# stevenabreu7/SparseRNNs

Measured on AMD Instinct MI355X. Metric: frames/sec at w8a16 S5 dim_scale=0.5 (NDNS shape), bit-exact vs CPU fxprun, higher is better.
Workload: dtype int32

## Files before the change

### include/s5fxp.h

```cpp
#ifndef S5FXP_H
#define S5FXP_H

#include <stddef.h>
#include <stdint.h>

#ifdef __cplusplus
extern "C" {
#endif

#define S5FXP_VERSION 115

enum {
    S5FXP_OK = 0,
    S5FXP_EBADARG = -1,
    S5FXP_ENEGSHIFT = -2,
    S5FXP_EUNSUPPORTED = -3,
    S5FXP_EHIP = -4,
    S5FXP_EWORKSPACE = -5
};

enum { S5FXP_FLOOR = 0, S5FXP_CEIL = 1, S5FXP_ROUND = 2 };

int s5fxp_version(void);
const char *s5fxp_strerror(int code);
// ... 114 lines not shown
typedef struct {
    s5fxp_norm_desc norm;
    s5fxp_ssm_desc ssm;
    s5fxp_dense_desc out2;
    int32_t l_bits, l_exp, r_bits, r_exp, res_bits, res_exp;
    int32_t sig_x_exp, sig_y_exp;
    int32_t lut[8];
} s5fxp_layer_desc;

typedef struct {
    int32_t n_layers;
    s5fxp_dense_desc encoder;
    const s5fxp_layer_desc *layers;
    s5fxp_dense_desc decoder;
} s5fxp_model_desc;

typedef struct s5fxp_model s5fxp_model;

typedef struct {
    int32_t *pre_s5;
    int32_t *u;
    int32_t *Bu_re, *Bu_im;
    int32_t *xs_re, *xs_im;
    int32_t *ys;
    int32_t *out2;
    int32_t *out2_sigmoid;
    int32_t *post_GLU;
    int32_t *residadd;
} s5fxp_layer_trace;

size_t s5fxp_model_blob_bytes(const s5fxp_model_desc *desc);

enum { S5FXP_MODEL_DEFAULT = 0, S5FXP_MODEL_FORCE_DENSE = 1, S5FXP_MODEL_FORCE_CSR = 2, S5FXP_MODEL_FORCE_GENERIC = 4,
       S5FXP_MODEL_NO_RESID_FOLD = 8, S5FXP_MODEL_NO_RESID_LAZY = 16, S5FXP_MODEL_NO_GATE_EXT = 32 };
int s5fxp_model_create(const s5fxp_model_desc *desc, void *dev_blob, size_t blob_bytes, int flags, void *stream,
                       s5fxp_model **out);
void s5fxp_model_destroy(s5fxp_model *m);

size_t s5fxp_workspace_bytes(const s5fxp_model *m, int B, int L);

#define S5FXP_STATUS_WORDS 128
enum { S5FXP_PATH_GENERIC = 1, S5FXP_PATH_FUSED = 2, S5FXP_PATH_STEP = 3, S5FXP_PATH_CLIP = 4 };
enum {
    S5FXP_ST_NEGSHIFT = 1,
    S5FXP_ST_NEGEXP = 2,
    S5FXP_ST_WIDE_STATE = 4,
    S5FXP_ST_WIDE_INPUT = 8,
    S5FXP_ST_REDO = 16
};

enum { S5FXP_FWD_DEFER_REDO = 1, S5FXP_FWD_EXACT = 2, S5FXP_FWD_NO_PAIR = 4 };

typedef int (*s5fxp_allreduce_max_fn)(void *ctx, float *dev_vals, int n, void *stream);

typedef struct {
    s5fxp_allreduce_max_fn allreduce;
    void *allreduce_ctx;
    void **scan_events;
    int32_t flags;
    const int32_t *state_in;
    int32_t *state_out;
    int32_t groups;
    void **gate_events;
} s5fxp_forward_opts;

int s5fxp_model_forward(const s5fxp_model *m, const int32_t *x, int x_bits, int x_exp, int B, int L, int32_t *y,
                        void *workspace, size_t workspace_bytes, int32_t *status, const s5fxp_layer_trace *traces,
// ... 102 lines not shown
```

### sparsernns_amd/_lib.py

```python
from __future__ import annotations

import ctypes as C
import os

import torch

_HERE = os.path.dirname(os.path.abspath(__file__))
LIB_PATH = os.environ.get("S5FXP_LIB") or os.path.join(_HERE, "libs5fxp.so")

I32P = C.POINTER(C.c_int32)
VOIDP = C.c_void_p

S5FXP_OK, S5FXP_EBADARG, S5FXP_ENEGSHIFT, S5FXP_EUNSUPPORTED, S5FXP_EHIP, S5FXP_EWORKSPACE = 0, -1, -2, -3, -4, -5
ST_NEGSHIFT, ST_NEGEXP, ST_WIDE_STATE, ST_WIDE_INPUT, ST_REDO = 1, 2, 4, 8, 16
FWD_DEFER_REDO, FWD_EXACT, FWD_NO_PAIR = 1, 2, 4
STATUS_WORDS = 128
PATH_GENERIC, PATH_FUSED, PATH_STEP, PATH_CLIP = 1, 2, 3, 4
STEP_MAX_ROWS = 32
STREAM_MAX_HOPS = 32
PUSH_FRESH, PUSH_ZEROS, PUSH_FINAL = 1, 2, 4
MODEL_DEFAULT, MODEL_FORCE_DENSE, MODEL_FORCE_CSR, MODEL_FORCE_GENERIC, MODEL_NO_RESID_FOLD, MODEL_NO_RESID_LAZY = 0, 1, 2, 4, 8, 16
MODEL_NO_GATE_EXT = 32


class DenseDesc(C.Structure):
    _fields_ = [("K", C.c_int32), ("M", C.c_int32), ("weight", I32P), ("bias", I32P)] + [
        (n, C.c_int32) for n in ("w_bits", "w_exp", "b_bits", "b_exp", "inp_bits", "inp_exp", "out_bits", "out_exp")]


class SSMDesc(C.Structure):
    _fields_ = [("H", C.c_int32), ("P", C.c_int32)] + [
        (n, I32P) for n in ("A_re", "A_im", "B_re", "B_im", "C_re", "C_im", "D")] + [
        (n, C.c_int32) for n in (
            "A_re_bits", "A_re_exp", "A_im_bits", "A_im_exp", "B_re_bits", "B_re_exp", "B_im_bits", "B_im_exp",
            "C_re_bits", "C_re_exp", "C_im_bits", "C_im_exp", "D_bits", "D_exp",
            "u_bits", "u_exp", "Bu_re_bits", "Bu_re_exp", "Bu_im_bits", "Bu_im_exp",
            "x_re_bits", "x_re_exp", "x_im_bits", "x_im_exp", "y_bits", "y_exp")]


class NormDesc(C.Structure):
    _fields_ = [(n, I32P) for n in ("minus_mean", "invsq_var", "scale", "bias")] + [
        (n, C.c_int32) for n in ("mean_bits", "mean_exp", "invsq_var_bits", "invsq_var_exp", "scale_bits",
                                 "scale_exp", "bias_bits", "bias_exp")]


class LayerDesc(C.Structure):
    _fields_ = [("norm", NormDesc), ("ssm", SSMDesc), ("out2", DenseDesc)] + [
        (n, C.c_int32) for n in ("l_bits", "l_exp", "r_bits", "r_exp", "res_bits", "res_exp", "sig_x_exp",
                                 "sig_y_exp")] + [("lut", C.c_int32 * 8)]


class ModelDesc(C.Structure):
    _fields_ = [("n_layers", C.c_int32), ("encoder", DenseDesc), ("layers", C.POINTER(LayerDesc)),
                ("decoder", DenseDesc)]

# ... 158 lines not shown
```

### sparsernns_amd/csrc/mfma_bn.hpp

```cpp
#pragma once
#include "mfma_proj.hpp"

namespace s5 {

struct StatusInit {
    int32_t path;
    int32_t rk[15];
    int32_t slots[15];
    int32_t stream[15];
};
__global__ __launch_bounds__(256) void k_clear2(int32_t *a, int na, int32_t *b, int nb, StatusInit si, int n_layers, GroupOff go)
{
    gshift(a, (int64_t)blockIdx.y * go.status);
    gshift(b, (int64_t)blockIdx.y * go.ws);
    for (int i = blockIdx.x * 256 + threadIdx.x; i < na + nb; i += gridDim.x * 256) {
        if (i < na) {
            int32_t v = 0;
            if (i == 2) v = si.path;
            else if (i >= 8 && (i & 7) == 5 && (i - 8) / 8 < n_layers) v = si.rk[(i - 8) / 8];
            else if (i >= 8 && (i & 7) == 6 && (i - 8) / 8 < n_layers) v = si.slots[(i - 8) / 8];
            else if (i >= 8 && (i & 7) == 7 && (i - 8) / 8 < n_layers) v = si.stream[(i - 8) / 8];
            a[i] = v;
        } else b[i - na] = 0;
    }
// ... 681 lines not shown
{
    v4i u;
#pragma unroll
    for (int k = 0; k < 4; ++k) {
        if constexpr (ARM == ROW_GENERIC) {
            int32_t o[2];
#pragma unroll
            for (int e = 0; e < 2; ++e) {
                const int32_t xe = e ? x[k] >> 16 : (int32_t)(int16_t)(x[k] & 0xffff);
                const int32_t me = e ? (int32_t)p.m[k] >> 16 : (int32_t)(int16_t)(p.m[k] & 0xffffu);
                const int32_t ie = e ? (int32_t)p.iv[k] >> 16 : (int32_t)(int16_t)(p.iv[k] & 0xffffu);
                const int32_t v = sat(asr(wshl(wadd(sat(wshl(xe, p.shx1), p.xb), me), p.l1), p.r1), p.b1);
                const int32_t t = sat(asr(__mul24(v, ie), p.rs2), p.b2);
                o[e] = sat(asr(wshl(t, p.cl), p.cr), p.cbits);
            }
            u[k] = (int32_t)(((uint32_t)o[0] & 0xffffu) | ((uint32_t)o[1] << 16));
        } else {
            const uint32_t xs = pk_mul_sat_u((uint32_t)x[k], p.mulx);
            int32_t t0, t1;
            if constexpr (ARM == ROW_PACKED) {
                const uint32_t v = pk_add_sat(xs, p.m[k]);
                t0 = mul24_hh<0>(v, p.iv[k]); t1 = mul24_hh<1>(v, p.iv[k]);
            } else {
                const int32_t v0 = asr(add_hh<0>(xs, p.m[k]), p.r1), v1 = asr(add_hh<1>(xs, p.m[k]), p.r1);
                t0 = mul24_h<0>(v0, p.iv[k]); t1 = mul24_h<1>(v1, p.iv[k]);
            }
            const uint32_t t = pk_cvt(asr(t0, p.rs2), asr(t1, p.rs2));
            u[k] = (int32_t)pk_ashr_u(pk_mul_sat_u(t, p.mulc), p.crp);
        }
    }
    return u;
}

struct BprojM2Args {
    BnArgs bn;
    const int16_t *x;
    MfmaW w;
    int32_t *bq;
    int16_t *u;
    int32_t *tr_bu_re, *tr_bu_im, *tr_pre_s5, *tr_u;
    int64_t N;
    int32_t L, TB, H, P;
    int32_t rs_re, rs_im, bre_bits, bim_bits, sh_re, sh_im;
    int32_t t_lo, t_len;
    int32_t k_re;
    int32_t no_u;
    int32_t live_slots;
    const float *ext;
    int32_t ext_reps;
    int32_t *status, *status_exps;
    const LayerDyn *lazy;
};

}
```

### sparsernns_amd/csrc/proj_p.hpp

```cpp
#pragma once
#ifdef S5_PHASE_PROF
__device__ long long g_phase_prof[2048 * 8];
#define PHASE_DECL unsigned prof_last, prof_a0 = 0, prof_a1 = 0, prof_a2 = 0, prof_a3 = 0, prof_a4 = 0, prof_a5 = 0, prof_a6 = 0, prof_a7 = 0; \
    { unsigned long long t_; asm volatile("s_memtime %0\n\ts_waitcnt lgkmcnt(0)" : "=s"(t_)); prof_last = __builtin_amdgcn_readfirstlane((unsigned)t_); }
#define PHASE_MARK(i, reg) do { unsigned long long t_; asm volatile("v_cmp_eq_u32 vcc, %1, %1\n\ts_nop 0\n\ts_memtime %0\n\ts_waitcnt lgkmcnt(0)" : "=s"(t_) : "v"(reg) : "memory", "vcc"); \
    const unsigned tl_ = __builtin_amdgcn_readfirstlane((unsigned)t_); prof_a##i = __builtin_amdgcn_readfirstlane(prof_a##i + (tl_ - prof_last)); prof_last = tl_; } while (0)
#define PHASE_DUMP do { if (threadIdx.x == 0 && blockIdx.x < 2048) { long long *o_ = g_phase_prof + blockIdx.x * 8; o_[0] = prof_a0; o_[1] = prof_a1; o_[2] = prof_a2; o_[3] = prof_a3; \
    o_[4] = prof_a4; o_[5] = prof_a5; o_[6] = prof_a6; o_[7] = prof_a7; } } while (0)
#else
#define PHASE_DECL
#define PHASE_MARK(i, reg)
#define PHASE_DUMP
#endif
#include "mfma_bn.hpp"

namespace s5 {

__host__ __device__ constexpr int shape_channels(int NT) { return (NT == 2 || NT == 5) ? 32 * NT - 16 : 32 * NT; }

template <int HC, int HP, int KP>
__device__ __forceinline__ void zero_plane_tail(int8_t *base, int rows)
{
    if constexpr (HC != HP) {
        static_assert(HP - HC == 16, "half a tile");
        for (int i = threadIdx.x; i < rows; i += blockDim.x) *reinterpret_cast<v4i *>(base + i * KP + HC) = v4i{0, 0, 0, 0};
    }
}

__device__ __forceinline__ void planes8_from_i32(const int32_t (&v)[8], v2i &hi, v2i &lo)
{
#pragma unroll
    for (int j = 0; j < 2; ++j) {
        const unsigned p01 = perm((unsigned)v[4 * j + 1], (unsigned)v[4 * j], 0x05010400u);
        const unsigned p23 = perm((unsigned)v[4 * j + 3], (unsigned)v[4 * j + 2], 0x05010400u);
        lo[j] = (int)(perm(p23, p01, 0x05040100u) ^ 0x80808080u);
        hi[j] = (int)perm(p23, p01, 0x07060302u);
    }
}

struct StepRange {
    int32_t t_lo, t_len;
};
template <int FT = 64>
__device__ __forceinline__ void tile_of(int64_t tile, const StepRange &sr, int64_t &b, int &t, int &nvalid)
{
    const int tps = (sr.t_len + FT - 1) / FT;
    b = tile / tps;
    const int tt = (int)(tile - b * tps) * FT;
    t = sr.t_lo + tt;
    nvalid = sr.t_len - tt < FT ? sr.t_len - tt : FT;
}

template <int FT = 64>
struct TileWalk {
    int tps, db, dti;
    int b, ti;
    __device__ __forceinline__ TileWalk(int64_t tile0, const StepRange &sr, unsigned step)
    {
        tps = (sr.t_len + FT - 1) / FT;
        db = (int)(step / (unsigned)tps); dti = (int)(step % (unsigned)tps);
        b = (int)((unsigned)tile0 / (unsigned)tps); ti = (int)((unsigned)tile0 % (unsigned)tps);
    }
    __device__ __forceinline__ void advance()
    {
        b += db; ti += dti;
        if (ti >= tps) { ti -= tps; ++b; }
    }
    __device__ __forceinline__ TileWalk next() const { TileWalk n = *this; n.advance(); return n; }
    __device__ __forceinline__ int t(const StepRange &sr) const { return sr.t_lo + ti * FT; }
// ... 24 lines not shown
    const int wct = wave % NC, wsub = wave / NC;
    const StepRange sr{a.t_lo, a.t_len};
    const int64_t tiles = (a.N / a.L) * ((sr.t_len + FT - 1) / FT);
    int64_t tile = blockIdx.x;

    v4i raw[NV];
    auto fetch = [&](const TileWalk<FT> &tw) {
        const int64_t b = tw.b;
        const int t = tw.t(sr), nv = tw.nvalid(sr);
        const char *xb = reinterpret_cast<const char *>(a.x + (b * a.L + t) * H);
#pragma unroll
        for (int i = 0; i < NV; ++i) {
            const int v = threadIdx.x + NTHR * i;
            int f = v / VPF;
            f = f < nv ? f : nv - 1;
            raw[i] = *reinterpret_cast<const v4i *>(xb + 2u * (unsigned)(f * H + 8 * (v % VPF)));
        }
    };
    TileWalk<FT> walk(tile, sr, gridDim.x);
    if (tile < tiles) fetch(walk);
    v4i wreg[NCT][KS];
    int32_t csv[NCT];
#pragma unroll
    for (int c = 0; c < NCT; ++c) {
        const int col = 32 * (wct + NC * c) + r;
        csv[c] = a.w.cs128[col];
#pragma unroll
        for (int ks = 0; ks < KS; ++ks)
            wreg[c][ks] = *reinterpret_cast<const v4i *>(a.w.wt + (size_t)col * a.w.Kp + 32 * ks + 16 * h);
    }
    const LayerDyn d = a.ext ? bn_finalize_mm_body(a.bn, a.ext, H, const_cast<LayerDyn *>(a.bn.dyn), a.status, a.status_exps, a.bn.xe.get(), a.ext_reps,
                                                   blockIdx.x == 0)
                             : *a.bn.dyn;
    const Bn16 bn = bn16_setup(a.bn, d, tab, H);
    constexpr bool LAZY = KS == 3 && !TRACE;
    ResolveU16 rz{};
    int lazy_arm = 0;
    if constexpr (LAZY) {
        if (a.lazy) {
            gshift_nn(a.lazy, (int64_t)blockIdx.y * go.ws);
            rz = resolve_u16_setup(a.lazy->res.post);
            lazy_arm = 1 + rz.arm;
        }
    }
    __syncthreads();

    prologue_loads_done();
    for (int it = 0; tile < tiles; tile += gridDim.x, ++it, walk.advance()) {
        const int64_t b0 = walk.b;
        const int t0 = walk.t(sr), nvalid = walk.nvalid(sr);
        const int64_t n0 = b0 * a.L + t0;
        char *ub = reinterpret_cast<char *>(a.u + n0 * H);
        int8_t *xh = Xh + (it & 1) * PLANE, *xl = Xl + (it & 1) * PLANE;
#pragma unroll
        for (int i = 0; i < NV; ++i) {
            const int v = threadIdx.x + NTHR * i, f = v / VPF, og = v % VPF;
            const int64_t n = n0 + f;
            int32_t xin[8], t[8], u[8];
            if constexpr (LAZY) {
                if (lazy_arm == 1 + RES_RIGHT) {
#pragma unroll
                    for (int e = 0; e < 4; ++e) raw[i][e] = (int)resolve_u16_pair<RES_RIGHT>(rz, (uint32_t)raw[i][e]);
                } else if (lazy_arm) {
#pragma unroll
                    for (int e = 0; e < 4; ++e) raw[i][e] = (int)resolve_u16_pair<RES_GENERIC>(rz, (uint32_t)raw[i][e]);
                }
            }
            unpack8_i16(raw[i], xin);
            bn16_x4(bn, reinterpret_cast<const int32_t(&)[4]>(xin[0]), 8 * og, reinterpret_cast<int32_t(&)[4]>(t[0]),
                    reinterpret_cast<int32_t(&)[4]>(u[0]));
            bn16_x4(bn, reinterpret_cast<const int32_t(&)[4]>(xin[4]), 8 * og + 4, reinterpret_cast<int32_t(&)[4]>(t[4]),
                    reinterpret_cast<int32_t(&)[4]>(u[4]));
            if (f < nvalid && (TRACE || !a.no_u)) {
                const v2i p0 = pack4_i16(u[0], u[1], u[2], u[3]), p1 = pack4_i16(u[4], u[5], u[6], u[7]);
                *reinterpret_cast<v4i *>(ub + 2u * (unsigned)(f * H + 8 * og)) = v4i{p0[0], p0[1], p1[0], p1[1]};
                if (TRACE) {
#pragma unroll
                    for (int e = 0; e < 8; ++e) {
                        if (a.tr_pre_s5) a.tr_pre_s5[n * H + 8 * og + e] = t[e];
                        if (a.tr_u) a.tr_u[n * H + 8 * og + e] = u[e];
                    }
                }
            }
            v2i hi, lo;
            planes8_from_i32(u, hi, lo);
            *reinterpret_cast<v2i *>(xh + f * KP + 8 * og) = hi;
            *reinterpret_cast<v2i *>(xl + f * KP + 8 * og) = lo;
        }
        if (tile + gridDim.x < tiles) fetch(walk.next());
        __syncthreads();
#pragma unroll
        for (int c = 0; c < NCT; ++c) {
            const int col = 32 * (wct + NC * c) + r;
            const int cc = SM >= 2 ? (r >> 4) : (col >= PC ? 1 : 0), p = SM >= 2 ? 16 * (wct + NC * c) + (r & 15) : col - cc * PC;
            const int rs = cc ? a.rs_im : a.rs_re, bits = cc ? a.bim_bits : a.bre_bits, sh = cc ? a.sh_im : a.sh_re;
            const int lsh = sh < 0 ? -sh : 0, rsh = sh > 0 ? sh : 0;
            SatB sbu;
            sbu.hi = (int32_t)((1u << (bits - 1)) - 1u); sbu.lo = ~sbu.hi;
            asm volatile("" : "+v"(sbu.lo), "+v"(sbu.hi));
#pragma unroll
            for (int sub0 = 0; sub0 < 2; sub0 += SUB0_STEP) {
                const int sub = sub0 + wsub;
                if (SUB0_STEP > 2 && sub >= 2) break;
                const int8_t *rowh = xh + (32 * sub + r) * KP + 16 * h, *rowl = xl + (32 * sub + r) * KP + 16 * h;
                v16i acc;
#pragma unroll
                for (int i = 0; i < 16; ++i) acc[i] = 0;
#pragma unroll
                for (int ks = 0; ks < KS; ++ks)
                    acc = __builtin_amdgcn_mfma_i32_32x32x32_i8(*reinterpret_cast<const v4i *>(rowh + 32 * ks), wreg[c][ks], acc, 0, 0, 0);
#pragma unroll
                for (int i = 0; i < 16; ++i) acc[i] = wadd(wshl(acc[i], 8), csv[c]);
#pragma unroll
                for (int ks = 0; ks < KS; ++ks)
                    acc = __builtin_amdgcn_mfma_i32_32x32x32_i8(*reinterpret_cast<const v4i *>(rowl + 32 * ks), wreg[c][ks], acc, 0, 0, 0);
#pragma unroll
                for (int g = 0; g < 4; ++g) {
                    const int o = 32 * sub + 8 * g + 4 * h;
                    const bool live = o < nvalid;
                    {
                        v4i q;
#pragma unroll
                        for (int e = 0; e < 4; ++e) {
                            const int32_t bu = sat(asr(acc[4 * g + e], rs), sbu);
                            q[e] = asr(wshl(bu, lsh), rsh);
                            if (TRACE && o + e < nvalid) {
                                if (!cc && a.tr_bu_re) a.tr_bu_re[(n0 + o + e) * PC + p] = bu;
                                if (cc && a.tr_bu_im) a.tr_bu_im[(n0 + o + e) * PC + p] = bu;
                            }
                        }
                        if (SM == 3) {
                            const int32_t o0 = __builtin_amdgcn_ds_swizzle(q[0], 0x401f), o2 = __builtin_amdgcn_ds_swizzle(q[2], 0x401f);
                            const v2i item = pack4_i16(o0, o2, q[1], q[3]);
                            if (live && (a.live_slots <= 0 || p < a.live_slots)) {
                                char *qb = reinterpret_cast<char *>(reinterpret_cast<int16_t *>(a.bq) + pair16_half(b0, t0 >> 2, 0, 0, a.TB, PC));
                                const unsigned qo = 2u * (unsigned)((((((p >> 5) * (a.TB >> 1) + (o >> 3)) << 6) + 2 * (p & 31) + cc) * 8) + 4 * ((o >> 2) & 1));
                                *reinterpret_cast<v2i *>(qb + qo) = item;
                            }
                        } else if (SM == 2) {
                            const int32_t kc = cc ? 0 : a.k_re;
                            const int32_t k0 = wadd(wshl(q[0], 16), kc), k2 = wadd(wshl(q[2], 16), kc);
                            v4i item;
                            item[0] = __builtin_amdgcn_ds_swizzle(k0, 0x401f);
                            item[1] = __builtin_amdgcn_ds_swizzle(k2, 0x401f);
                            item[2] = wadd(wshl(q[1], 16), kc);
                            item[3] = wadd(wshl(q[3], 16), kc);
                            if (live) *reinterpret_cast<v4i *>(a.bq + pair_word(b0, (t0 + o) >> 2, p, a.TB, PC) + 4 * cc) = item;
                        } else if (SM == 1) {
                            if (live && (a.live_slots <= 0 || p < a.live_slots))
                                *reinterpret_cast<v2i *>(reinterpret_cast<int16_t *>(a.bq) + native_word(b0, t0 + o, p, cc, a.TB, PC)) =
                                    pack4_i16(q[0], q[1], q[2], q[3]);
                        } else if (live)
                            *reinterpret_cast<v4i *>(a.bq + native_word(b0, t0 + o, p, cc, a.TB, PC)) = q;
                    }
                }
            }
        }
    }
}

using v2u16 = __attribute__((ext_vector_type(2))) unsigned short;

struct CfgOp {
    int l, r, b;
    SatB sb;
    __device__ __forceinline__ int32_t operator()(int32_t d) const { return sat(asr(wshl(d, l), r), sb); }
};
__device__ __forceinline__ CfgOp make_cfg(bool on, int bits, int e, int bits2, int e2)
{
    CfgOp c;
    c.l = on && e2 > e ? e2 - e : 0;
    c.r = on && e > e2 ? e - e2 : 0;
    const int b1 = on && e2 != e ? bits : 32, b2 = on && bits > bits2 ? bits2 : 32;
    c.b = b1 < b2 ? b1 : b2;
    c.sb = sat_bounds(c.b);
    return c;
}

template <int KSTEPS>
__device__ __forceinline__ void mfma_planes(v16i &acc, const v4i (&w)[KSTEPS], const int8_t *rowh, const int8_t *rowl,
                                            const int32_t *cs)
{
#pragma unroll
    for (int i = 0; i < 16; ++i) acc[i] = 0;
#pragma unroll
    for (int ks = 0; ks < KSTEPS; ++ks)
        acc = __builtin_amdgcn_mfma_i32_32x32x32_i8(w[ks], *reinterpret_cast<const v4i *>(rowh + 32 * ks), acc, 0, 0, 0);
#pragma unroll
    for (int g = 0; g < 4; ++g) {
// ... 86 lines not shown
```

### sparsernns_amd/csrc/s5fxp_fast.hpp

```cpp
#pragma once

namespace s5 {
struct StepParams;
}

struct MfmaWDev {
    MfmaW w{};
    const int32_t *bias_eff = nullptr;
};

struct FastLayer {
    MfmaWDev bproj, cre, cim, out2;
    MfmaWDev bproj_pair;
    const int32_t *Dpad = nullptr;
    const int32_t *sigtab = nullptr;
    const int16_t *sigdir = nullptr;
    int sigdir_bits = 0;
    bool bias16 = false;
    bool compact_ok = false;
    int n_live = 0;
    int c_slots = 0;
    MfmaWDev c_bproj, c_bproj_pair, c_cre, c_cim;
    ScanBounds c_bounds;
    const int32_t *c_a_re = nullptr, *c_a_im = nullptr;
// ... 263 lines not shown
}

bool fast_bn_ext(const s5fxp_model *m)
{
    bool bn_ext = !m->cfg.no_bn_ext && m->enc.out_bits <= 16 && m->enc.out_exp >= 0 && m->enc.out_exp <= 15;
    for (int li = 0; li < m->n_layers; ++li) {
        const s5fxp_norm_desc &n = m->layers[li].nd;
        auto ok = [](int bits, int e) { return bits <= 16 && e >= 0 && e <= 15; };
        bn_ext = bn_ext && ok(n.mean_bits, n.mean_exp) && ok(n.invsq_var_bits, n.invsq_var_exp) &&
                 (!m->layers[li].scale || ok(n.scale_bits, n.scale_exp)) && (!m->layers[li].nbias || ok(n.bias_bits, n.bias_exp)) &&
                 m->layers[li].res_bits <= 16;
    }
    return bn_ext;
}

enum GateForm { GATE_TRACED, GATE_FT64, GATE_FT32, GATE_GBN };

struct LayerPlan {
    bool compact;
    Rung rung;
    int P;
    int ks;
    int live_slots;
    int stream_slots;
    int32_t bound;
    int32_t xmax;
    bool direct;
    bool pk16;
    bool gate_bn;
    bool gate_urec;
    bool resid_fold;
    bool resid_lazy;
    bool gate_ext;
    GateForm gate;
    const MfmaW *w_bproj, *w_cre, *w_cim;
    const int32_t *a_re, *a_im;
};

LayerPlan plan_layer(const s5fxp_model *m, int li, int fwd_flags, bool traced, bool carry, bool fold)
{
    const LayerDev &l = m->layers[li];
    const FastLayer &fl = m->fast->layers[li];
    const s5fxp_ssm_desc &s = l.sd;
    const FastShape sh = fast_shape(m->H, m->P);
    LayerPlan p{};
    p.compact = fl.compact_ok && !m->cfg.no_compact && !traced && !carry;
    p.rung = select_rung(m, li, fwd_flags, traced, p.compact);
    const Rung &r = p.rung;
    p.P = p.compact ? fl.c_slots : m->P;
    p.ks = p.P / 32;
    p.live_slots = stream_live_slots(m, li, r, p.compact);
    p.stream_slots = p.live_slots ? p.live_slots : p.P;
    const ScanBounds &cb = fl.c_bounds;
    p.bound = r.pair ? (p.compact ? cb.pair_xmax : l.pair_xmax) : (p.compact ? cb.quad_xmax : l.quad_xmax);
    p.xmax = 32767;
    if (r.quad) p.xmax = std::min(p.bound, p.xmax);
    if (r.quad && r.s16 && !r.pair) p.xmax = std::min(p.xmax, 32766);
    const bool out2_conv = s.y_bits > l.out2.inp_bits || s.y_exp > l.out2.inp_exp;
    p.direct = r.s16 && fl.sigdir_bits > 0;
    p.pk16 = p.direct && !traced && !m->cfg.no_pk16 && fl.bias16 && s.y_bits == 16 && l.out2.out_bits == 16 && l.res_bits == 16 &&
             l.l_bits == 16 && !out2_conv && l.l_exp - s.y_exp <= 14;
    p.gate_bn = p.pk16 && fold && sh.gate32 && m->cfg.gate_bn;
    p.gate = traced ? GATE_TRACED : p.gate_bn ? GATE_GBN : (sh.gate32 && p.pk16 && !m->cfg.cgate_ft64) ? GATE_FT32 : GATE_FT64;
    p.gate_urec = p.gate == GATE_FT32 && fold && !l.scale && !l.nbias && !m->cfg.no_gate_urec;
    p.w_bproj = r.pair ? &(p.compact ? fl.c_bproj_pair : fl.bproj_pair).w : &(p.compact ? fl.c_bproj : fl.bproj).w;
    p.w_cre = &(p.compact ? fl.c_cre : fl.cre).w;
    p.w_cim = &(p.compact ? fl.c_cim : fl.cim).w;
    p.a_re = p.compact ? fl.c_a_re : l.a_re;
    p.a_im = p.compact ? fl.c_a_im : l.a_im;
    return p;
}

LayerPlan plain_plan(const s5fxp_model *m, int li) { return plan_layer(m, li, S5FXP_FWD_DEFER_REDO, false, false, fast_bn_ext(m)); }

template <int NT, class Kernel> auto ks_kernel(int ks, Kernel kernel)
{
    if constexpr (NT == 2) return kernel(std::integral_constant<int, 1>{});
    else if constexpr (NT == 5) return kernel(std::integral_constant<int, 3>{});
    else {
        if constexpr (NT == 6)
            if (ks == 4) return kernel(std::integral_constant<int, 4>{});
        return ks == 1 ? kernel(std::integral_constant<int, 1>{}) : kernel(std::integral_constant<int, 2>{});
    }
}
template <int NT> constexpr int bproj_waves_of() { return NT == 2 ? 2 : NT == 3 ? 4 : NT == 5 ? 6 : 8; }

template <int SM> auto bproj_kernel(const FastShape &sh, int ks)
{
    return nt_kernel(sh.nt, [&](auto n) {
        constexpr int NT = decltype(n)::value;
        return ks_kernel<NT>(ks, [](auto k) { return k_bproj_p<NT, bproj_waves_of<NT>(), false, SM, 2 * decltype(k)::value>; });
    });
}
inline auto bproj_traced_kernel(const FastShape &sh)
{
    return nt_kernel(sh.nt, [](auto n) { constexpr int NT = decltype(n)::value; return k_bproj_p<NT, bproj_waves_of<NT>(), true>; });
}
// ... 181 lines not shown
    }

    int bn_exponents(int li, const BnArgs &bn) const
    {
        LayerDyn *d = dyn + li;
        if (!bn_ext) {
            const unsigned rg = std::min(ew_grid(NH / 4), 2048u);
            return bn_exponent_ops([&](auto op) {
                hipLaunchKernelGGL(k_bn_reduce16<decltype(op)::value>, dim3(rg), dim3(256), 0, st, bn, (const int16_t *)h, NH, H, d);
            }, bn, d, status, status_exps(li), opts, st);
        }
        if (!fold) {
            if (allreduce && allreduce(opts->allreduce_ctx, ext(li), 2 * H, (void *)st)) return S5FXP_EHIP;
            hipLaunchKernelGGL(k_bn_finalize_mm, dim3(1), dim3(256), 0, st, bn, (const float *)ext(li), H, d, status, status_exps(li));
        }
        return S5FXP_OK;
    }

    void bproj(int li, const BnArgs &bn) const
    {
        const LayerPlan &p = layer[li];
        const s5fxp_ssm_desc &s = m->layers[li].sd;
        const s5fxp_layer_trace *tr = trace(li);
        BprojM2Args a{};
        a.bn = bn; a.x = h; a.w = *p.w_bproj; a.bq = I32(w.bq); a.u = I16(w.u);
        a.tr_bu_re = tr ? tr->Bu_re : nullptr; a.tr_bu_im = tr ? tr->Bu_im : nullptr;
        a.tr_pre_s5 = tr ? tr->pre_s5 : nullptr; a.tr_u = tr ? tr->u : nullptr;
        a.N = N; a.L = L; a.TB = w.TB; a.H = H; a.P = p.P;
        a.rs_re = s.u_exp + s.B_re_exp - s.Bu_re_exp; a.rs_im = s.u_exp + s.B_im_exp - s.Bu_im_exp;
        a.bre_bits = s.Bu_re_bits; a.bim_bits = s.Bu_im_bits; a.sh_re = s.Bu_re_exp - s.x_re_exp; a.sh_im = s.Bu_im_exp - s.x_im_exp;
        a.k_re = 65536 - (1 << (16 - s.A_re_exp));
        a.live_slots = p.live_slots;
        a.no_u = (p.gate_bn || p.gate_urec) && defer ? 1 : 0;
        if (fold) {
            a.ext = ext(li);
            a.ext_reps = EXT_REPS; a.status = status; a.status_exps = status_exps(li);
        }
        a.lazy = h_lazy;
        a.t_lo = 0; a.t_len = L;
        const size_t smem = 16 * (size_t)sh.hp + 4 * 64 * (size_t)(sh.hp + 16);
        const Rung &r = p.rung;
        auto kernel = tr ? bproj_traced_kernel(sh)
                         : r.pairl ? bproj_kernel<3>(sh, p.ks) : r.pair ? bproj_kernel<2>(sh, p.ks) : r.s16 ? bproj_kernel<1>(sh, p.ks) : bproj_kernel<0>(sh, p.ks);
        launch(kernel, grid_bproj, 64 * sh.bproj_waves, smem, nullptr, nullptr, a);
    }
    ScanQuadArgs quad_args(int li, const int32_t *run_if) const
    {
        const LayerPlan &p = layer[li];
        const s5fxp_ssm_desc &s = m->layers[li].sd;
        ScanQuadArgs q{};
        q.bq = I32(w.bq); q.xs = I32(w.xs); q.a_re = p.a_re; q.a_im = p.a_im; q.B = B; q.TB = w.TB; q.P = p.P;
        q.ea_re = s.A_re_exp; q.ea_im = s.A_im_exp; q.run_if = run_if; q.x0_re = x0(li, 0); q.x0_im = x0(li, 1);
        q.live_slots = p.live_slots;
        if (!run_if) q.cc = carry_check(li);
        return q;
    }
    CarryCheck carry_check(int li) const
    {
        const LayerPlan &p = layer[li];
        CarryCheck c{};
        if (!state_in || !p.rung.quad) return c;
        c.xmax = p.xmax; c.bad_bits = ST_WIDE_STATE | (defer ? ST_REDO : 0); c.redo = &dyn[li].redo; c.status = status;
        return c;
    }
    const int32_t *x0(int li, int c) const
    {
// ... 219 lines not shown
```

Measured before the change: 764.9 million.

## Add packed 16-bit BN row path and packed Bu epilogue to bproj kernel

For the KS==3 untraced bproj kernel, adds a specialized batch-norm path that processes 8 channels per row using packed 16-bit ops (bn16_row8) with a precomputed per-channel table. It also adds a packed-pair epilogue that converts, clips and shifts Bu outputs two at a time with v_pk_min/max/lshl instead of per-element 32-bit saturation. The tile loop moves into an include file instantiated per row arm, which grows code size and register pressure. A model flag can disable the new path.

```diff
diff --git a/include/s5fxp.h b/include/s5fxp.h
--- a/include/s5fxp.h
+++ b/include/s5fxp.h
@@ -170,7 +170,7 @@
 size_t s5fxp_model_blob_bytes(const s5fxp_model_desc *desc);
 
 enum { S5FXP_MODEL_DEFAULT = 0, S5FXP_MODEL_FORCE_DENSE = 1, S5FXP_MODEL_FORCE_CSR = 2, S5FXP_MODEL_FORCE_GENERIC = 4,
-       S5FXP_MODEL_NO_RESID_FOLD = 8, S5FXP_MODEL_NO_RESID_LAZY = 16, S5FXP_MODEL_NO_GATE_EXT = 32 };
+       S5FXP_MODEL_NO_RESID_FOLD = 8, S5FXP_MODEL_NO_RESID_LAZY = 16, S5FXP_MODEL_NO_GATE_EXT = 32, S5FXP_MODEL_NO_BPROJ_ROW8 = 64 };
 int s5fxp_model_create(const s5fxp_model_desc *desc, void *dev_blob, size_t blob_bytes, int flags, void *stream,
                        s5fxp_model **out);
 void s5fxp_model_destroy(s5fxp_model *m);
diff --git a/sparsernns_amd/_lib.py b/sparsernns_amd/_lib.py
--- a/sparsernns_amd/_lib.py
+++ b/sparsernns_amd/_lib.py
@@ -21,6 +21,7 @@
 PUSH_FRESH, PUSH_ZEROS, PUSH_FINAL = 1, 2, 4
 MODEL_DEFAULT, MODEL_FORCE_DENSE, MODEL_FORCE_CSR, MODEL_FORCE_GENERIC, MODEL_NO_RESID_FOLD, MODEL_NO_RESID_LAZY = 0, 1, 2, 4, 8, 16
 MODEL_NO_GATE_EXT = 32
+MODEL_NO_BPROJ_ROW8 = 64
 
 
 class DenseDesc(C.Structure):
diff --git a/sparsernns_amd/csrc/mfma_bn.hpp b/sparsernns_amd/csrc/mfma_bn.hpp
--- a/sparsernns_amd/csrc/mfma_bn.hpp
+++ b/sparsernns_amd/csrc/mfma_bn.hpp
@@ -737,6 +737,51 @@
     return u;
 }
 
+enum { BPK_NONE = 0, BPK_CVT = 1, BPK_CLIP = 2 };
+struct BuPk {
+    int32_t s;
+    uint32_t lo, hi, lsh;
+};
+__host__ __device__ __forceinline__ int bu_pk_arm1(int rs, int bits, int sh)
+{
+    const int lsh = sh < 0 ? -sh : 0, rsh = sh > 0 ? sh : 0;
+    if (rs < 0 || rs + rsh > 31 || bits - rsh < 1 || bits - rsh + lsh > 16) return BPK_NONE;
+    return bits - rsh == 16 && lsh == 0 ? BPK_CVT : BPK_CLIP;
+}
+__host__ __device__ __forceinline__ int bu_pk_arm(int rs_re, int bre_bits, int sh_re, int rs_im, int bim_bits, int sh_im)
+{
+    const int a = bu_pk_arm1(rs_re, bre_bits, sh_re), b = bu_pk_arm1(rs_im, bim_bits, sh_im);
+    return a == BPK_NONE || b == BPK_NONE ? BPK_NONE : a == BPK_CVT && b == BPK_CVT ? BPK_CVT : BPK_CLIP;
+}
+__host__ __device__ __forceinline__ BuPk bu_pk_setup(int rs, int bits, int sh)
+{
+    const int lsh = sh < 0 ? -sh : 0, rsh = sh > 0 ? sh : 0;
+    const uint32_t top = (1u << ((bits - rsh - 1) & 15)) - 1u;
+    BuPk p;
+    p.s = rs + rsh;
+    p.hi = 0x10001u * top; p.lo = 0x10001u * (~top & 0xffffu); p.lsh = 0x10001u * (uint32_t)(lsh & 15);
+    return p;
+}
+__device__ __forceinline__ uint32_t pk_min(uint32_t a, uint32_t b)
+{
+    uint32_t r;
+    asm("v_pk_min_i16 %0, %1, %2" : "=v"(r) : "v"(a), "v"(b));
+    return r;
+}
+__device__ __forceinline__ uint32_t pk_lshl(uint32_t a, uint32_t s)
+{
+    uint32_t r;
+    asm("v_pk_lshlrev_b16 %0, %1, %2" : "=v"(r) : "v"(s), "v"(a));
+    return r;
+}
+template <int ARM>
+__device__ __forceinline__ uint32_t bu_pk_pair(const BuPk &p, int32_t a0, int32_t a1)
+{
+    const uint32_t t = pk_cvt(asr(a0, p.s), asr(a1, p.s));
+    if constexpr (ARM == BPK_CVT) return t;
+    else return pk_lshl(pk_max(pk_min(t, p.hi), p.lo), p.lsh);
+}
+
 struct BprojM2Args {
     BnArgs bn;
     const int16_t *x;
@@ -751,6 +796,7 @@
     int32_t k_re;
     int32_t no_u;
     int32_t live_slots;
+    int32_t no_row8;
     const float *ext;
     int32_t ext_reps;
     int32_t *status, *status_exps;
diff --git a/sparsernns_amd/csrc/proj_bproj_tiles.inc b/sparsernns_amd/csrc/proj_bproj_tiles.inc
--- /dev/null
+++ b/sparsernns_amd/csrc/proj_bproj_tiles.inc
@@ -0,0 +1,174 @@
+    __syncthreads();
+
+    prologue_loads_done();
+    for (int it = 0; tile < tiles; tile += gridDim.x, ++it, walk.advance()) {
+        const int64_t b0 = walk.b;
+        const int t0 = walk.t(sr), nvalid = walk.nvalid(sr);
+        const int64_t n0 = b0 * a.L + t0;
+        char *ub = reinterpret_cast<char *>(a.u + n0 * H);
+        int8_t *xh = Xh + (it & 1) * PLANE, *xl = Xl + (it & 1) * PLANE;
+        if constexpr (RA != ROW_GENERIC) {
+            int tid = threadIdx.x;
+            asm volatile("" : "+v"(tid));
+#pragma unroll
+            for (int i = 0; i < NV; ++i) {
+                const int v = tid + NTHR * i, f = v / VPF, og = v % VPF;
+                if (lazy_arm == 1 + RES_RIGHT) {
+#pragma unroll
+                    for (int e = 0; e < 4; ++e) raw[i][e] = (int)resolve_u16_pair<RES_RIGHT>(rz, (uint32_t)raw[i][e]);
+                } else if (lazy_arm) {
+#pragma unroll
+                    for (int e = 0; e < 4; ++e) raw[i][e] = (int)resolve_u16_pair<RES_GENERIC>(rz, (uint32_t)raw[i][e]);
+                }
+                const v4i bm = reinterpret_cast<const v4i *>(tab)[2 * og], bi = reinterpret_cast<const v4i *>(tab)[2 * og + 1];
+                Bn16Row br = brow;
+#pragma unroll
+                for (int k = 0; k < 4; ++k) { br.m[k] = (uint32_t)bm[k]; br.iv[k] = (uint32_t)bi[k]; }
+                const v4i uv = bn16_row8<RA>(br, raw[i]);
+                if (f < nvalid && !a.no_u) *reinterpret_cast<v4i *>(ub + 2u * (unsigned)(f * H + 8 * og)) = uv;
+                v2i hi, lo;
+                planes8_from_pairs(uv, hi, lo);
+                *reinterpret_cast<v2i *>(xh + f * KP + 8 * og) = hi;
+                *reinterpret_cast<v2i *>(xl + f * KP + 8 * og) = lo;
+            }
+        } else {
+#pragma unroll
+            for (int i = 0; i < NV; ++i) {
+                const int v = threadIdx.x + NTHR * i, f = v / VPF, og = v % VPF;
+                const int64_t n = n0 + f;
+                int32_t xin[8], t[8], u[8];
+                if constexpr (LAZY) {
+                    if (lazy_arm == 1 + RES_RIGHT) {
+#pragma unroll
+                        for (int e = 0; e < 4; ++e) raw[i][e] = (int)resolve_u16_pair<RES_RIGHT>(rz, (uint32_t)raw[i][e]);
+                    } else if (lazy_arm) {
+#pragma unroll
+                        for (int e = 0; e < 4; ++e) raw[i][e] = (int)resolve_u16_pair<RES_GENERIC>(rz, (uint32_t)raw[i][e]);
+                    }
+                }
+                unpack8_i16(raw[i], xin);
+                bn16_x4(bn, reinterpret_cast<const int32_t(&)[4]>(xin[0]), 8 * og, reinterpret_cast<int32_t(&)[4]>(t[0]),
+                        reinterpret_cast<int32_t(&)[4]>(u[0]));
+                bn16_x4(bn, reinterpret_cast<const int32_t(&)[4]>(xin[4]), 8 * og + 4, reinterpret_cast<int32_t(&)[4]>(t[4]),
+                        reinterpret_cast<int32_t(&)[4]>(u[4]));
+                if (f < nvalid && (TRACE || !a.no_u)) {
+                    const v2i p0 = pack4_i16(u[0], u[1], u[2], u[3]), p1 = pack4_i16(u[4], u[5], u[6], u[7]);
+                    *reinterpret_cast<v4i *>(ub + 2u * (unsigned)(f * H + 8 * og)) = v4i{p0[0], p0[1], p1[0], p1[1]};
+                    if (TRACE) {
+#pragma unroll
+                        for (int e = 0; e < 8; ++e) {
+                            if (a.tr_pre_s5) a.tr_pre_s5[n * H + 8 * og + e] = t[e];
+                            if (a.tr_u) a.tr_u[n * H + 8 * og + e] = u[e];
+                        }
+                    }
+                }
+                v2i hi, lo;
+                planes8_from_i32(u, hi, lo);
+                *reinterpret_cast<v2i *>(xh + f * KP + 8 * og) = hi;
+                *reinterpret_cast<v2i *>(xl + f * KP + 8 * og) = lo;
+            }
+        }
+        if (tile + gridDim.x < tiles) fetch(walk.next());
+        __syncthreads();
+#pragma unroll
+        for (int c = 0; c < NCT; ++c) {
+            const int col = 32 * (wct + NC * c) + r;
+            const int cc = SM >= 2 ? (r >> 4) : (col >= PC ? 1 : 0), p = SM >= 2 ? 16 * (wct + NC * c) + (r & 15) : col - cc * PC;
+            const int rs = cc ? a.rs_im : a.rs_re, bits = cc ? a.bim_bits : a.bre_bits, sh = cc ? a.sh_im : a.sh_re;
+            const int lsh = sh < 0 ? -sh : 0, rsh = sh > 0 ? sh : 0;
+            SatB sbu;
+            sbu.hi = (int32_t)((1u << (bits - 1)) - 1u); sbu.lo = ~sbu.hi;
+            asm volatile("" : "+v"(sbu.lo), "+v"(sbu.hi));
+#pragma unroll
+            for (int sub0 = 0; sub0 < 2; sub0 += SUB0_STEP) {
+                const int sub = sub0 + wsub;
+                if (SUB0_STEP > 2 && sub >= 2) break;
+                const int8_t *rowh = xh + (32 * sub + r) * KP + 16 * h, *rowl = xl + (32 * sub + r) * KP + 16 * h;
+                v16i acc;
+#pragma unroll
+                for (int i = 0; i < 16; ++i) acc[i] = 0;
+#pragma unroll
+                for (int ks = 0; ks < KS; ++ks)
+                    acc = __builtin_amdgcn_mfma_i32_32x32x32_i8(*reinterpret_cast<const v4i *>(rowh + 32 * ks), wreg[c][ks], acc, 0, 0, 0);
+#pragma unroll
+                for (int i = 0; i < 16; ++i) acc[i] = wadd(wshl(acc[i], 8), csv[c]);
+#pragma unroll
+                for (int ks = 0; ks < KS; ++ks)
+                    acc = __builtin_amdgcn_mfma_i32_32x32x32_i8(*reinterpret_cast<const v4i *>(rowl + 32 * ks), wreg[c][ks], acc, 0, 0, 0);
+                if constexpr (PKB && RA != ROW_GENERIC) {
+                    {
+                        auto epilogue_pairs = [&](auto arm_c, const BuPk &bp) {
+                            constexpr int ARM = decltype(arm_c)::value;
+#pragma unroll
+                            for (int g = 0; g < 4; ++g) {
+                                const int o = 32 * sub + 8 * g + 4 * h;
+                                if constexpr (SM == 3) {
+                                    const uint32_t q02 = bu_pk_pair<ARM>(bp, acc[4 * g], acc[4 * g + 2]), q13 = bu_pk_pair<ARM>(bp, acc[4 * g + 1], acc[4 * g + 3]);
+                                    const v2i item = {__builtin_amdgcn_ds_swizzle((int)q02, 0x401f), (int)q13};
+                                    if (o < nvalid && (a.live_slots <= 0 || p < a.live_slots)) {
+                                        char *qb = reinterpret_cast<char *>(reinterpret_cast<int16_t *>(a.bq) + pair16_half(b0, t0 >> 2, 0, 0, a.TB, PC));
+                                        const unsigned qo = 2u * (unsigned)((((((p >> 5) * (a.TB >> 1) + (o >> 3)) << 6) + 2 * (p & 31) + cc) * 8) + 4 * ((o >> 2) & 1));
+                                        *reinterpret_cast<v2i *>(qb + qo) = item;
+                                    }
+                                } else {
+                                    const uint32_t q01 = bu_pk_pair<ARM>(bp, acc[4 * g], acc[4 * g + 1]), q23 = bu_pk_pair<ARM>(bp, acc[4 * g + 2], acc[4 * g + 3]);
+                                    if (o < nvalid && (a.live_slots <= 0 || p < a.live_slots))
+                                        *reinterpret_cast<v2i *>(reinterpret_cast<int16_t *>(a.bq) + native_word(b0, t0 + o, p, cc, a.TB, PC)) = v2i{(int)q01, (int)q23};
+                                }
+                            }
+                        };
+                        if (pb_arm == BPK_CVT) {
+                            BuPk bp{};
+                            bp.s = rs + rsh;
+                            epilogue_pairs(std::integral_constant<int, BPK_CVT>{}, bp);
+                        } else {
+                            int shv = sh;
+                            asm volatile("" : "+v"(shv));
+                            epilogue_pairs(std::integral_constant<int, BPK_CLIP>{}, bu_pk_setup(rs, bits, shv));
+                        }
+                        continue;
+                    }
+                }
+#pragma unroll
+                for (int g = 0; g < 4; ++g) {
+                    const int o = 32 * sub + 8 * g + 4 * h;
+                    const bool live = o < nvalid;
+                    {
+                        v4i q;
+#pragma unroll
+                        for (int e = 0; e < 4; ++e) {
+                            const int32_t bu = sat(asr(acc[4 * g + e], rs), sbu);
+                            q[e] = asr(wshl(bu, lsh), rsh);
+                            if (TRACE && o + e < nvalid) {
+                                if (!cc && a.tr_bu_re) a.tr_bu_re[(n0 + o + e) * PC + p] = bu;
+                                if (cc && a.tr_bu_im) a.tr_bu_im[(n0 + o + e) * PC + p] = bu;
+                            }
+                        }
+                        if (SM == 3) {
+                            const int32_t o0 = __builtin_amdgcn_ds_swizzle(q[0], 0x401f), o2 = __builtin_amdgcn_ds_swizzle(q[2], 0x401f);
+                            const v2i item = pack4_i16(o0, o2, q[1], q[3]);
+                            if (live && (a.live_slots <= 0 || p < a.live_slots)) {
+                                char *qb = reinterpret_cast<char *>(reinterpret_cast<int16_t *>(a.bq) + pair16_half(b0, t0 >> 2, 0, 0, a.TB, PC));
+                                const unsigned qo = 2u * (unsigned)((((((p >> 5) * (a.TB >> 1) + (o >> 3)) << 6) + 2 * (p & 31) + cc) * 8) + 4 * ((o >> 2) & 1));
+                                *reinterpret_cast<v2i *>(qb + qo) = item;
+                            }
+                        } else if (SM == 2) {
+                            const int32_t kc = cc ? 0 : a.k_re;
+                            const int32_t k0 = wadd(wshl(q[0], 16), kc), k2 = wadd(wshl(q[2], 16), kc);
+                            v4i item;
+                            item[0] = __builtin_amdgcn_ds_swizzle(k0, 0x401f);
+                            item[1] = __builtin_amdgcn_ds_swizzle(k2, 0x401f);
+                            item[2] = wadd(wshl(q[1], 16), kc);
+                            item[3] = wadd(wshl(q[3], 16), kc);
+                            if (live) *reinterpret_cast<v4i *>(a.bq + pair_word(b0, (t0 + o) >> 2, p, a.TB, PC) + 4 * cc) = item;
+                        } else if (SM == 1) {
+                            if (live && (a.live_slots <= 0 || p < a.live_slots))
+                                *reinterpret_cast<v2i *>(reinterpret_cast<int16_t *>(a.bq) + native_word(b0, t0 + o, p, cc, a.TB, PC)) =
+                                    pack4_i16(q[0], q[1], q[2], q[3]);
+                        } else if (live)
+                            *reinterpret_cast<v4i *>(a.bq + native_word(b0, t0 + o, p, cc, a.TB, PC)) = q;
+                    }
+                }
+            }
+        }
+    }
diff --git a/sparsernns_amd/csrc/proj_p.hpp b/sparsernns_amd/csrc/proj_p.hpp
--- a/sparsernns_amd/csrc/proj_p.hpp
+++ b/sparsernns_amd/csrc/proj_p.hpp
@@ -13,6 +13,7 @@
 #define PHASE_DUMP
 #endif
 #include "mfma_bn.hpp"
+#include <type_traits>
 
 namespace s5 {
 
@@ -35,6 +36,16 @@
         const unsigned p23 = perm((unsigned)v[4 * j + 3], (unsigned)v[4 * j + 2], 0x05010400u);
         lo[j] = (int)(perm(p23, p01, 0x05040100u) ^ 0x80808080u);
         hi[j] = (int)perm(p23, p01, 0x07060302u);
+    }
+}
+
+__device__ __forceinline__ void planes8_from_pairs(const v4i &u, v2i &hi, v2i &lo)
+{
+#pragma unroll
+    for (int j = 0; j < 2; ++j) {
+        const unsigned p01 = (unsigned)u[2 * j], p23 = (unsigned)u[2 * j + 1];
+        lo[j] = (int)(perm(p23, p01, 0x06040200u) ^ 0x80808080u);
+        hi[j] = (int)perm(p23, p01, 0x07050301u);
     }
 }
 
@@ -125,7 +136,23 @@
     const LayerDyn d = a.ext ? bn_finalize_mm_body(a.bn, a.ext, H, const_cast<LayerDyn *>(a.bn.dyn), a.status, a.status_exps, a.bn.xe.get(), a.ext_reps,
                                                    blockIdx.x == 0)
                              : *a.bn.dyn;
-    const Bn16 bn = bn16_setup(a.bn, d, tab, H);
+    constexpr bool ROW8 = KS == 3 && !TRACE;
+    constexpr bool PKB = ROW8 && (SM == 1 || SM == 3);
+    Bn16Row brow{};
+    int row_arm = ROW_GENERIC, pb_arm = BPK_NONE;
+    if constexpr (ROW8) {
+        if (!a.no_row8 && !a.bn.scale && !a.bn.bias) {
+            const int de = a.bn.ue - d.bn_e;
+            bn16_row_shifts(brow, a.bn.xb, a.bn.mb, a.bn.ib, a.bn.b1, a.bn.b2, a.bn.out_bits < a.bn.ub ? a.bn.out_bits : a.bn.ub,
+                            __builtin_amdgcn_readfirstlane(d.bn1.shx), __builtin_amdgcn_readfirstlane(d.bn1.post),
+                            __builtin_amdgcn_readfirstlane(d.rs2), __builtin_amdgcn_readfirstlane(de));
+            row_arm = brow.arm;
+        }
+        if constexpr (PKB) {
+            pb_arm = bu_pk_arm(a.rs_re, a.bre_bits, a.sh_re, a.rs_im, a.bim_bits, a.sh_im);
+            if (pb_arm == BPK_NONE) row_arm = ROW_GENERIC;
+        }
+    }
     constexpr bool LAZY = KS == 3 && !TRACE;
     ResolveU16 rz{};
     int lazy_arm = 0;
@@ -136,118 +163,28 @@
             lazy_arm = 1 + rz.arm;
         }
     }
-    __syncthreads();
-
-    prologue_loads_done();
-    for (int it = 0; tile < tiles; tile += gridDim.x, ++it, walk.advance()) {
-        const int64_t b0 = walk.b;
-        const int t0 = walk.t(sr), nvalid = walk.nvalid(sr);
-        const int64_t n0 = b0 * a.L + t0;
-        char *ub = reinterpret_cast<char *>(a.u + n0 * H);
-        int8_t *xh = Xh + (it & 1) * PLANE, *xl = Xl + (it & 1) * PLANE;
-#pragma unroll
-        for (int i = 0; i < NV; ++i) {
-            const int v = threadIdx.x + NTHR * i, f = v / VPF, og = v % VPF;
-            const int64_t n = n0 + f;
-            int32_t xin[8], t[8], u[8];
-            if constexpr (LAZY) {
-                if (lazy_arm == 1 + RES_RIGHT) {
-#pragma unroll
-                    for (int e = 0; e < 4; ++e) raw[i][e] = (int)resolve_u16_pair<RES_RIGHT>(rz, (uint32_t)raw[i][e]);
-                } else if (lazy_arm) {
-#pragma unroll
-                    for (int e = 0; e < 4; ++e) raw[i][e] = (int)resolve_u16_pair<RES_GENERIC>(rz, (uint32_t)raw[i][e]);
-                }
-            }
-            unpack8_i16(raw[i], xin);
-            bn16_x4(bn, reinterpret_cast<const int32_t(&)[4]>(xin[0]), 8 * og, reinterpret_cast<int32_t(&)[4]>(t[0]),
-                    reinterpret_cast<int32_t(&)[4]>(u[0]));
-            bn16_x4(bn, reinterpret_cast<const int32_t(&)[4]>(xin[4]), 8 * og + 4, reinterpret_cast<int32_t(&)[4]>(t[4]),
-                    reinterpret_cast<int32_t(&)[4]>(u[4]));
-            if (f < nvalid && (TRACE || !a.no_u)) {
-                const v2i p0 = pack4_i16(u[0], u[1], u[2], u[3]), p1 = pack4_i16(u[4], u[5], u[6], u[7]);
-                *reinterpret_cast<v4i *>(ub + 2u * (unsigned)(f * H + 8 * og)) = v4i{p0[0], p0[1], p1[0], p1[1]};
-                if (TRACE) {
-#pragma unroll
-                    for (int e = 0; e < 8; ++e) {
-                        if (a.tr_pre_s5) a.tr_pre_s5[n * H + 8 * og + e] = t[e];
-                        if (a.tr_u) a.tr_u[n * H + 8 * og + e] = u[e];
-                    }
-                }
-            }
-            v2i hi, lo;
-            planes8_from_i32(u, hi, lo);
-            *reinterpret_cast<v2i *>(xh + f * KP + 8 * og) = hi;
-            *reinterpret_cast<v2i *>(xl + f * KP + 8 * og) = lo;
-        }
-        if (tile + gridDim.x < tiles) fetch(walk.next());
-        __syncthreads();
-#pragma unroll
-        for (int c = 0; c < NCT; ++c) {
-            const int col = 32 * (wct + NC * c) + r;
-            const int cc = SM >= 2 ? (r >> 4) : (col >= PC ? 1 : 0), p = SM >= 2 ? 16 * (wct + NC * c) + (r & 15) : col - cc * PC;
-            const int rs = cc ? a.rs_im : a.rs_re, bits = cc ? a.bim_bits : a.bre_bits, sh = cc ? a.sh_im : a.sh_re;
-            const int lsh = sh < 0 ? -sh : 0, rsh = sh > 0 ? sh : 0;
-            SatB sbu;
-            sbu.hi = (int32_t)((1u << (bits - 1)) - 1u); sbu.lo = ~sbu.hi;
-            asm volatile("" : "+v"(sbu.lo), "+v"(sbu.hi));
-#pragma unroll
-            for (int sub0 = 0; sub0 < 2; sub0 += SUB0_STEP) {
-                const int sub = sub0 + wsub;
-                if (SUB0_STEP > 2 && sub >= 2) break;
-                const int8_t *rowh = xh + (32 * sub + r) * KP + 16 * h, *rowl = xl + (32 * sub + r) * KP + 16 * h;
-                v16i acc;
-#pragma unroll
-                for (int i = 0; i < 16; ++i) acc[i] = 0;
-#pragma unroll
-                for (int ks = 0; ks < KS; ++ks)
-                    acc = __builtin_amdgcn_mfma_i32_32x32x32_i8(*reinterpret_cast<const v4i *>(rowh + 32 * ks), wreg[c][ks], acc, 0, 0, 0);
-#pragma unroll
-                for (int i = 0; i < 16; ++i) acc[i] = wadd(wshl(acc[i], 8), csv[c]);
-#pragma unroll
-                for (int ks = 0; ks < KS; ++ks)
-                    acc = __builtin_amdgcn_mfma_i32_32x32x32_i8(*reinterpret_cast<const v4i *>(rowl + 32 * ks), wreg[c][ks], acc, 0, 0, 0);
-#pragma unroll
-                for (int g = 0; g < 4; ++g) {
-                    const int o = 32 * sub + 8 * g + 4 * h;
-                    const bool live = o < nvalid;
-                    {
-                        v4i q;
-#pragma unroll
-                        for (int e = 0; e < 4; ++e) {
-                            const int32_t bu = sat(asr(acc[4 * g + e], rs), sbu);
-                            q[e] = asr(wshl(bu, lsh), rsh);
-                            if (TRACE && o + e < nvalid) {
-                                if (!cc && a.tr_bu_re) a.tr_bu_re[(n0 + o + e) * PC + p] = bu;
-                                if (cc && a.tr_bu_im) a.tr_bu_im[(n0 + o + e) * PC + p] = bu;
-                            }
-                        }
-                        if (SM == 3) {
-                            const int32_t o0 = __builtin_amdgcn_ds_swizzle(q[0], 0x401f), o2 = __builtin_amdgcn_ds_swizzle(q[2], 0x401f);
-                            const v2i item = pack4_i16(o0, o2, q[1], q[3]);
-                            if (live && (a.live_slots <= 0 || p < a.live_slots)) {
-                                char *qb = reinterpret_cast<char *>(reinterpret_cast<int16_t *>(a.bq) + pair16_half(b0, t0 >> 2, 0, 0, a.TB, PC));
-                                const unsigned qo = 2u * (unsigned)((((((p >> 5) * (a.TB >> 1) + (o >> 3)) << 6) + 2 * (p & 31) + cc) * 8) + 4 * ((o >> 2) & 1));
-                                *reinterpret_cast<v2i *>(qb + qo) = item;
-                            }
-                        } else if (SM == 2) {
-                            const int32_t kc = cc ? 0 : a.k_re;
-                            const int32_t k0 = wadd(wshl(q[0], 16), kc), k2 = wadd(wshl(q[2], 16), kc);
-                            v4i item;
-                            item[0] = __builtin_amdgcn_ds_swizzle(k0, 0x401f);
-                            item[1] = __builtin_amdgcn_ds_swizzle(k2, 0x401f);
-                            item[2] = wadd(wshl(q[1], 16), kc);
-                            item[3] = wadd(wshl(q[3], 16), kc);
-                            if (live) *reinterpret_cast<v4i *>(a.bq + pair_word(b0, (t0 + o) >> 2, p, a.TB, PC) + 4 * cc) = item;
-                        } else if (SM == 1) {
-                            if (live && (a.live_slots <= 0 || p < a.live_slots))
-                                *reinterpret_cast<v2i *>(reinterpret_cast<int16_t *>(a.bq) + native_word(b0, t0 + o, p, cc, a.TB, PC)) =
-                                    pack4_i16(q[0], q[1], q[2], q[3]);
-                        } else if (live)
-                            *reinterpret_cast<v4i *>(a.bq + native_word(b0, t0 + o, p, cc, a.TB, PC)) = q;
-                    }
-                }
-            }
+    if constexpr (!ROW8) {
+        constexpr int RA = ROW_GENERIC;
+        const Bn16 bn = bn16_setup(a.bn, d, tab, H);
+#include "proj_bproj_tiles.inc"
+    } else if (row_arm == ROW_GENERIC) {
+        constexpr int RA = ROW_GENERIC;
+        const Bn16 bn = bn16_setup(a.bn, d, tab, H);
+#include "proj_bproj_tiles.inc"
+    } else {
+        [[maybe_unused]] const Bn16 bn{};
+        uint32_t *rt = reinterpret_cast<uint32_t *>(tab);
+        for (int i = threadIdx.x; i < H / 2; i += NTHR) {
+            const int32_t m0 = sat(wshl(a.bn.mm[2 * i], d.bn1.shy), a.bn.mb), m1 = sat(wshl(a.bn.mm[2 * i + 1], d.bn1.shy), a.bn.mb);
+            rt[8 * (i >> 2) + (i & 3)] = ((uint32_t)m0 & 0xffffu) | ((uint32_t)m1 << 16);
+            rt[8 * (i >> 2) + 4 + (i & 3)] = ((uint32_t)a.bn.isv[2 * i] & 0xffffu) | ((uint32_t)a.bn.isv[2 * i + 1] << 16);
+        }
+        if (row_arm == ROW_PACKED) {
+            constexpr int RA = ROW_PACKED;
+#include "proj_bproj_tiles.inc"
+        } else {
+            constexpr int RA = ROW_SHIFTED;
+#include "proj_bproj_tiles.inc"
         }
     }
 }
diff --git a/sparsernns_amd/csrc/s5fxp_fast.hpp b/sparsernns_amd/csrc/s5fxp_fast.hpp
--- a/sparsernns_amd/csrc/s5fxp_fast.hpp
+++ b/sparsernns_amd/csrc/s5fxp_fast.hpp
@@ -319,6 +319,7 @@
     bool resid_fold;
     bool resid_lazy;
     bool gate_ext;
+    bool bproj_row8;
     GateForm gate;
     const MfmaW *w_bproj, *w_cre, *w_cim;
     const int32_t *a_re, *a_im;
@@ -350,6 +351,7 @@
     p.gate_bn = p.pk16 && fold && sh.gate32 && m->cfg.gate_bn;
     p.gate = traced ? GATE_TRACED : p.gate_bn ? GATE_GBN : (sh.gate32 && p.pk16 && !m->cfg.cgate_ft64) ? GATE_FT32 : GATE_FT64;
     p.gate_urec = p.gate == GATE_FT32 && fold && !l.scale && !l.nbias && !m->cfg.no_gate_urec;
+    p.bproj_row8 = !(m->flags & S5FXP_MODEL_NO_BPROJ_ROW8);
     p.w_bproj = r.pair ? &(p.compact ? fl.c_bproj_pair : fl.bproj_pair).w : &(p.compact ? fl.c_bproj : fl.bproj).w;
     p.w_cre = &(p.compact ? fl.c_cre : fl.cre).w;
     p.w_cim = &(p.compact ? fl.c_cim : fl.cim).w;
@@ -597,6 +599,7 @@
         a.k_re = 65536 - (1 << (16 - s.A_re_exp));
         a.live_slots = p.live_slots;
         a.no_u = (p.gate_bn || p.gate_urec) && defer ? 1 : 0;
+        a.no_row8 = p.bproj_row8 ? 0 : 1;
         if (fold) {
             a.ext = ext(li);
             a.ext_reps = EXT_REPS; a.status = status; a.status_exps = status_exps(li);
```

New measurement: 774.5 million, median of 6. 1.01x the previous value.
